# Harrypotterrrr/DVD-GAN

Hardware: AMD Instinct MI355X
Metric: clips/sec per G+Ds+Dt step, 48x64x64 UCF-101 synth (higher is better)
Workload: dtype bf16; 1 GPU; UCF-101-shaped 101-class 48x64x64 clips, G+Ds+Dt hinge step, ch=32, k_sample=8, batch 64/GPU (BASELINE configs[1]); global_batch=64, parallelism=dp1

## Files before the change

dvd_gan_amd/csrc/conv_wgrad.hip:

```cpp
#include "conv_common.h"
#include "prof.h"
#include <cstdlib>
#include <type_traits>

namespace {

struct WgK {
    const char* x; const char* dy; float* dw;
    int M, C, ldx, Cin_real, Cout, Cy, ldy;
    int T, H, W, logH, logW, Hin, Win;
    int kt, kh, kw, up2, relu_in;
    int tiles_co, tiles_ci, rows_per_split;
    long long s_co, s_ci, s_tap;
    size_t x_bytes, dy_bytes;
    int maxshift, xcd_remap;
    float* dbias;
    float* wsb;
    float* ws;
    int fold, cout_f;
};

template <typename G>
__host__ __device__ __forceinline__ size_t ws_tile_off(size_t slice, G gx, int bx, int kw, int t, int tile_elems) { return ((slice * gx + bx) * kw + t) * (size_t)tile_elems; }
template <typename G>
__host__ __device__ __forceinline__ size_t ws_slice_stride(G gx, int kw, int tile_elems) { return ws_tile_off(1, gx, 0, kw, 0, tile_elems); }
template <typename N>
__host__ __device__ __forceinline__ size_t ws_bias_off(size_t slice, N n, int i, int BMc) { return (slice * n + i) * BMc; }

__device__ __forceinline__ void xcd_block_remap(const WgK& p, int& bx, int& bz) {
    bx = blockIdx.x; bz = blockIdx.z;
    if (p.xcd_remap) {
        const int gx = gridDim.x, total = gx * gridDim.z, lin = bx + gx * bz;
        const int xcd = lin & 7, qd = total >> 3, rr = total & 7;
        const int lp = (xcd < rr ? xcd * (qd + 1) : rr * (qd + 1) + (xcd - rr) * qd) + (lin >> 3);
        bz = lp / gx; bx = lp - bz * gx;
    }
}
__device__ __forceinline__ void bf16x8_unpack(const u32x4& r, float (&v)[8]) {
    v[0] = __uint_as_float(r.x << 16); v[1] = __uint_as_float(r.x & 0xffff0000u);
    v[2] = __uint_as_float(r.y << 16); v[3] = __uint_as_float(r.y & 0xffff0000u);
    v[4] = __uint_as_float(r.z << 16); v[5] = __uint_as_float(r.z & 0xffff0000u);
    v[6] = __uint_as_float(r.w << 16); v[7] = __uint_as_float(r.w & 0xffff0000u);
}
#define WG_BIAS_FINISH(CPRA, RPPA, NV, TAB, TO_WS, N, I)                                                                \
    do {                                                                                                                \
        __syncthreads();                                                                                                \
        if (tid < CPRA) {                                                                                               \
            for (int k = 0; k < NV; ++k) {                                                                              \
                float a = 0.f;                                                                                          \
                for (int r = 0; r < RPPA; ++r) a += TAB;                                                                \
                const int co = co0 + tid * NV + k;                                                                      \
                if (TO_WS) p.wsb[ws_bias_off(bz, N, I, BMc) + tid * NV + k] = a;                                        \
                else if (co < p.Cout && a != 0.f) atomicAdd(p.dbias + co, a);      \
            }                                                                                                           \
        }                                                                                                               \
        __syncthreads();                                                                                                \
    } while (0)
#define WG_TILE_TAIL(ACC, ROW0, COL0, KW_, T, TAP)                                                                      \
    do {                                                                                                                \
        _Pragma("unroll") for (int r = 0; r < 16; ++r)                                                                  \
            ep[((r & 3) + 8 * (r >> 2) + 4 * (lane >> 5)) * 32 + (lane & 31)] = ACC[r];                                 \
        __builtin_amdgcn_s_waitcnt(0xc07f);                                                                             \
        __builtin_amdgcn_wave_barrier();                                                                                \
        const int ci = ci0 + COL0 + (lane & 31);                                                                        \
        const int cob = co0 + ROW0 + (lane >> 5);                                                                       \
        const int wtap = TAP;                   \
        if (p.ws) {                                                                                                     \
            float* wt = p.ws + ws_tile_off(bz, gridDim.x, bx, KW_, T, BMc * BNc) + (size_t)(ROW0) * BNc + COL0;         \
            _Pragma("unroll 1") for (int j = 0; j < 16; ++j)                                                            \
                wt[(size_t)(2 * j + (lane >> 5)) * BNc + (lane & 31)] = ep[(2 * j + (lane >> 5)) * 32 + (lane & 31)];   \
        } else if (ci < p.Cin_real) {                                                                                   \
            float* dst = p.dw + ci * p.s_ci + wtap * p.s_tap;                                                           \
            _Pragma("unroll 1") for (int j = 0; j < 16; ++j) {                                                          \
                const int co = cob + 2 * j;                                                                             \
                const float v = ep[(2 * j + (lane >> 5)) * 32 + (lane & 31)];                                           \
                if (co < p.Cout && v != 0.f) atomicAdd(dst + co * p.s_co, v);                                           \
            }                                                                                                           \
        }                                                                                                               \
        __builtin_amdgcn_wave_barrier();                                                                                \
    } while (0)
template <typename T, int TA, int TB>
__global__ __launch_bounds__(NT) void conv_wgrad_kernel(WgK p) {
    constexpr bool kBf16 = sizeof(T) == 2;
    static_assert(kBf16 || (TA == 2 && TB == 2), "exact mode uses the 128 x 128 tile");
    constexpr int BKW = kBf16 ? 32 : 16;
    constexpr int BMc = TA * 64, BNc = TB * 64;
    constexpr int RSA = BMc * 2 + 64, RSB = BNc * 2 + 64;
    constexpr int TA_BYTES = kBf16 ? 32 * RSA : TILEB, TB_BYTES = kBf16 ? 32 * RSB : TILEB;
    __shared__ __attribute__((aligned(16))) char smem[2][TA_BYTES + TB_BYTES];
    const int tid = threadIdx.x, lane = tid & 63, wave = tid >> 6;
    const int wm = wave >> 1, wn = wave & 1;
    int bx, bz;
    xcd_block_remap(p, bx, bz);
    const int tiles = p.tiles_co * p.tiles_ci;
    const int tap = bx / tiles;
    const int rem = bx - tap * tiles;
    const int tco = rem / p.tiles_ci, tci = rem - tco * p.tiles_ci;
    const int co0 = tco * BMc, ci0 = tci * BNc;
    const int it = tap / (p.kh * p.kw), r2 = tap - it * p.kh * p.kw;
    const int iy = r2 / p.kw, ix = r2 - iy * p.kw;
    const int dt = it - (p.kt >> 1), dy_ = iy - (p.kh >> 1), dx = ix - (p.kw >> 1);
    const int m_begin = bz * p.rows_per_split;
    const int m_end = min(p.M, m_begin + p.rows_per_split);

    f32x16 acc[TA][TB];
    {
        const f32x16 zacc = {0.f, 0.f, 0.f, 0.f, 0.f, 0.f, 0.f, 0.f, 0.f, 0.f, 0.f, 0.f, 0.f, 0.f, 0.f, 0.f};
#pragma unroll
        for (int a = 0; a < TA; ++a)
#pragma unroll
            for (int b = 0; b < TB; ++b) acc[a][b] = zacc;
    }

    constexpr unsigned ESZ = sizeof(T);
    const int xbase_row = p.up2 ? (m_begin / (p.H * p.W)) * p.Hin * p.Win : max(0, m_begin - p.maxshift);
    const size_t xbase_b = (size_t)xbase_row * p.ldx * ESZ, ybase_b = (size_t)m_begin * p.ldy * ESZ;
    const size_t xleft = p.x_bytes - xbase_b, yleft = p.dy_bytes > ybase_b ? p.dy_bytes - ybase_b : 0;
    const __amdgpu_buffer_rsrc_t rx = __builtin_amdgcn_make_buffer_rsrc(
        (void*)(p.x + xbase_b), 0, xleft > 0xfffffffeull ? 0xfffffffeu : (unsigned)xleft, 0x00020000);
    const __amdgpu_buffer_rsrc_t rdy = __builtin_amdgcn_make_buffer_rsrc(
        (void*)(p.dy + ybase_b), 0, yleft > 0xfffffffeull ? 0xfffffffeu : (unsigned)yleft, 0x00020000);
    const int delta = (dt * p.H + dy_) * p.W + dx;
    auto xoff = [&](int m, unsigned chan_bytes, bool cvalid) __attribute__((always_inline)) -> unsigned {
        int fm, ym, xm;
        grid_pos(m, p.H, p.W, p.logH, p.logW, fm, ym, xm);
        const int xx = xm + dx, yy = ym + dy_;
        int tt = dt;
        if (p.kt > 1) tt += fm % p.T;
        const bool ok = cvalid && m < m_end && (unsigned)yy < (unsigned)p.H && (unsigned)xx < (unsigned)p.W &&
                        (unsigned)tt < (unsigned)p.T;
        int row = m + delta;
        if (p.up2) row = ((fm + dt) * p.Hin + (yy >> 1)) * p.Win + (xx >> 1);
        return ok ? (unsigned)(row - xbase_row) * ((unsigned)p.ldx * ESZ) + chan_bytes : 0xffffffffu;
    };
    auto yoff = [&](int m, unsigned chan_bytes, bool cvalid) __attribute__((always_inline)) -> unsigned {
        return (cvalid && m < m_end) ? (unsigned)(m - m_begin) * ((unsigned)p.ldy * ESZ) + chan_bytes : 0xffffffffu;
    };

    if constexpr (kBf16) {
        constexpr int CPRA = BMc / 8, RPPA = NT / CPRA, NPA = 32 / RPPA;
        constexpr int CPRB = BNc / 8, RPPB = NT / CPRB, NPB = 32 / RPPB;
        const int rra = tid / CPRA, cka = tid % CPRA, rrb = tid / CPRB, ckb = tid % CPRB;
        const int cy = co0 + cka * 8, cx = ci0 + ckb * 8;
        const bool cyv = cy < p.Cy, cxv = cx < p.C;
// ... 386 lines not shown
                xoffs[kb][hl][t] = TA_BYTES + wn * XHALF + fr * 64 + fcol2;
            }
    const int aoff = frow * RSA + fcol2 + (wm * 64) * 2;
    auto mma1 = [&](const char* st) __attribute__((always_inline)) {
        constexpr int NU = 2 * KW;
        bf16x8 fa[2][2], fb[NU];
        auto ldA = [&](int kb) __attribute__((always_inline)) {
#pragma unroll
            for (int a = 0; a < 2; ++a) {
                const char* pz = st + aoff + kb * 16 * RSA + a * 64;
                fa[kb][a] = tr2(pz, pz + 4 * RSA);
            }
        };
        auto ldB = [&](int u) __attribute__((always_inline)) {
            const int kb = u / KW, t = u % KW;
            if constexpr (UP2) fb[u] = tr2(st + xoffs[kb][0][t], st + xoffs[kb][1][t]);
            else fb[u] = tr2(st + xoffs[kb][0][0] + t * 64, st + xoffs[kb][1][0] + t * 64);
        };
        ldA(0); ldB(0); ldB(1);
        __builtin_amdgcn_sched_barrier(0);
#pragma unroll
        for (int u = 0; u < NU; ++u) {
            if (u + 2 < NU) ldB(u + 2);
            if (u == KW - 2) ldA(1);
            const int kb = u / KW, t = u % KW;
            acc[0][t] = __builtin_amdgcn_mfma_f32_32x32x16_bf16(fa[kb][0], fb[u], acc[0][t], 0, 0, 0);
            acc[1][t] = __builtin_amdgcn_mfma_f32_32x32x16_bf16(fa[kb][1], fb[u], acc[1][t], 0, 0, 0);
            __builtin_amdgcn_sched_barrier(0);
        }
    };
    auto mma = [&](int buf) __attribute__((always_inline)) {
#pragma unroll
        for (int s_ = 0; s_ < NS; ++s_) mma1(&smem[buf * STAGE + s_ * SUB]);
    };
    if (m_begin < m_end) {
        const bool late = NWAVE == 8 && NS == 2 && wave >= 4;
        gload(m_begin);
        lstore(0);
        if (late) gload(m_begin + 32 * NS);
        __builtin_amdgcn_s_waitcnt(0xc07f);
        __builtin_amdgcn_s_barrier();
        int buf = 0;
        for (int mk = m_begin; mk < m_end; mk += 32 * NS, buf ^= 1) {
            if (!late) {
                gload(mk + 32 * NS);
                mma(buf);
                lstore(buf ^ 1);
            } else {
                mma1(&smem[buf * STAGE]);
                lstore(buf ^ 1);
                gload(mk + 2 * 32 * NS);
                mma1(&smem[buf * STAGE + (NS - 1) * SUB]);
            }
            __builtin_amdgcn_s_waitcnt(0xc07f);
            __builtin_amdgcn_s_barrier();
        }
        __builtin_amdgcn_s_waitcnt(0x0070);
    }
    if (do_bias) {
        float* red = reinterpret_cast<float*>(&smem[0]);
#pragma unroll
        for (int k = 0; k < 8; ++k) red[tid * 8 + k] = bs[k];
        WG_BIAS_FINISH(CPRA, RPPA, 8, red[(r * CPRA + tid) * 8 + k], spread, gridDim.x, bx);
    }
    float* ep = reinterpret_cast<float*>(&smem[0]) + wave * (32 * 32);
#pragma unroll
    for (int a = 0; a < 2; ++a)
#pragma unroll
        for (int t = 0; t < KW; ++t)
            WG_TILE_TAIL(acc[a][t], wm * 64 + a * 32, wn * 32, KW, t, irow * KW + t);
}
template <int I, int N, typename F>
__device__ __forceinline__ void static_for(F&& f) {
    if constexpr (I < N) {
        f(std::integral_constant<int, I>{});
        static_for<I + 1, N>(f);
    }
}
template <bool V>
__device__ __forceinline__ void mfma_pinned(f32x16& c, const bf16x8& a, const bf16x8& b) {
    if constexpr (V) asm volatile("v_mfma_f32_32x32x16_bf16 %0, %1, %2, %0" : "+v"(c) : "v"(a), "v"(b));
    else asm volatile("v_mfma_f32_32x32x16_bf16 %0, %1, %2, %0" : "+a"(c) : "v"(a), "v"(b));
}

#ifndef DVD_EXP_ROW4
#define DVD_EXP_ROW4 0
#endif
template <int KW, int AW, int BW, int WCO, int WCI, bool RELU, int DEPTH = 2, bool FOLD = false>
__global__ __launch_bounds__(256) void conv_wgrad_row4_kernel(WgK p) {
    constexpr bool BLDS = KW == 3 && AW * BW * KW > 16 && DEPTH >= 2;
    static_assert(WCO * WCI == 4, "four waves, one per SIMD");
    constexpr int NTt = 256, BMc = WCO * AW * 32, NHB = WCI * BW, BNc = NHB * 32;
    constexpr int RSA = BMc * 2 + 64;
    constexpr int TA_BYTES = 32 * RSA;
    constexpr int XROWS = KW == 5 ? 64 : 48, XHALF = XROWS * 64, TB_BYTES = NHB * XHALF;
    constexpr int SUB = TA_BYTES + TB_BYTES;
    constexpr int EPIB = 4 * 32 * 32 * 4, REDB = NTt * 8 * 4;
    constexpr int LDSB0 = 3 * SUB > EPIB ? (3 * SUB > REDB ? 3 * SUB : REDB) : (EPIB > REDB ? EPIB : REDB);
    constexpr int LDSB = LDSB0 + (BLDS ? REDB : 0);
    __shared__ __attribute__((aligned(16))) char smem[LDSB];
    const int tid = threadIdx.x, lane = tid & 63, wave = tid >> 6;
    const int wm = wave / WCI, wn = wave % WCI;
    int bx = blockIdx.x, bz = blockIdx.z;
    if (p.xcd_remap) {
        const int gx = gridDim.x, total = gx * gridDim.z, lin = bx + gx * bz;
        const int xcd = lin & 7, qd = total >> 3, rr = total & 7;
        const int lp = (xcd < rr ? xcd * (qd + 1) : rr * (qd + 1) + (xcd - rr) * qd) + (lin >> 3);
        bz = lp / gx; bx = lp - bz * gx;
    }
    const int tiles = p.tiles_co * p.tiles_ci;
    const int irow = bx / tiles;
    const int rem = bx - irow * tiles;
    const int tco = rem / p.tiles_ci, tci = rem - tco * p.tiles_ci;
    const int co0 = tco * BMc, ci0 = tci * BNc;
    constexpr int pad = KW >> 1;
    static_assert(!FOLD || (KW == 3 && BMc == 128), "the folded form runs on the 3-tap 128-channel tile");
    const int it = FOLD ? 0 : irow / KW, iy = FOLD ? irow : irow - it * KW;
    const int dyl = FOLD ? ((co0 / p.cout_f) >> 1) - 1 + irow : iy - pad, dtl = FOLD ? 0 : it - (p.kt >> 1);
    const int m_begin = bz * p.rows_per_split;
    const int m_end = min(p.M, m_begin + p.rows_per_split);

    f32x16 acc[AW][BW][KW];
    {
        const f32x16 zacc = {0.f, 0.f, 0.f, 0.f, 0.f, 0.f, 0.f, 0.f, 0.f, 0.f, 0.f, 0.f, 0.f, 0.f, 0.f, 0.f};
#pragma unroll
        for (int a = 0; a < AW; ++a)
#pragma unroll
            for (int b = 0; b < BW; ++b)
#pragma unroll
                for (int t = 0; t < KW; ++t) acc[a][b][t] = zacc;
    }
    const int xbase_row = max(0, m_begin - p.maxshift);
    const int ybase_row = FOLD ? 4 * m_begin - 2 * (p.W > 32 ? m_begin & (p.W - 1) : 0) : m_begin;
    const size_t xbase_b = (size_t)xbase_row * p.ldx * 2, ybase_b = (size_t)ybase_row * p.ldy * 2;
    const size_t xleft = p.x_bytes - xbase_b, yleft = p.dy_bytes > ybase_b ? p.dy_bytes - ybase_b : 0;
    const __amdgpu_buffer_rsrc_t rx = __builtin_amdgcn_make_buffer_rsrc(
        (void*)(p.x + xbase_b), 0, xleft > 0xfffffffeull ? 0xfffffffeu : (unsigned)xleft, 0x00020000);
    const __amdgpu_buffer_rsrc_t rdy = __builtin_amdgcn_make_buffer_rsrc(
        (void*)(p.dy + ybase_b), 0, yleft > 0xfffffffeull ? 0xfffffffeu : (unsigned)yleft, 0x00020000);
    const int segw = min(p.W, 32), logsegw = min(p.logW, 5);
    const int fpr = segw + KW - 1, frows = (32 >> logsegw) * fpr;
    constexpr int CPRA = BMc / 8, RPPA = NTt / CPRA, NPA = 32 / RPPA;
    const int rra = tid / CPRA, cka = tid % CPRA;
    const int cy = co0 + cka * 8;
    const bool cyv = cy < p.Cy;
    constexpr int CPX = NHB * 4;
    constexpr int NXL = (XROWS * CPX + NTt - 1) / NTt;
    constexpr int NOPS = NPA + NXL;
    constexpr bool XFULL = NXL * NTt == XROWS * CPX;
    int xa[NXL];
    static_assert(NTt % CPX == 0, "chunk i of a thread sits NTt / CPX footprint rows below chunk i - 1");
    const int xdst0 = ((tid % CPX) >> 2) * XHALF + (tid / CPX) * 64 + ((tid % CPX) & 3) * 16;
    unsigned xld[NXL];
    bool xv[NXL];
    const bool twofr = (32 >> logsegw) > p.H;
    const bool wide = p.W > 32;
    const unsigned ldx2 = (unsigned)p.ldx * 2, ldy2 = (unsigned)p.ldy * 2;
#pragma unroll
    for (int i = 0; i < NXL; ++i) {
        const int q = tid + i * NTt, row = q / CPX, c8 = q % CPX;
        const int seg = row / fpr, j = row - seg * fpr;
        const int cx = ci0 + c8 * 8;
        const int fo = twofr ? seg >> p.logH : 0, yl = twofr ? seg & (p.H - 1) : seg;
        const int xya = yl + dyl, xxa = j - pad;
        xa[i] = wide ? xxa : xya;
        xv[i] = row < frows && cx < p.C && (wide || (unsigned)xxa < (unsigned)p.W);
        const int delta = (fo << (p.logW + p.logH)) + (xya << p.logW) + xxa;
        xld[i] = (unsigned)delta * ldx2 + (unsigned)cx * 2;
    }
    unsigned yld = (unsigned)rra * ldy2 + (unsigned)cy * 2;
    unsigned ystep = (unsigned)RPPA * ldy2;
    if constexpr (FOLD) {
        static_assert(!FOLD || RPPA == 16, "16 rows per staging pass");
        const int ph = cy / p.cout_f, c = cy - ph * p.cout_f, W2 = 2 * p.W;
        yld = (unsigned)(((rra >> logsegw) * 2 + (ph >> 1)) * W2 + 2 * (rra & (segw - 1)) + (ph & 1)) * ldy2 + (unsigned)c * 2;
        ystep = (unsigned)(segw == 32 ? 32 : (16 >> logsegw) * 2 * W2) * ldy2;
    }
    const int dt_rows = p.kt > 1 ? dtl << (p.logW + p.logH) : 0;
    u32x4 R[DEPTH][NOPS];
    struct Geo { int sval; unsigned xoff, yoff; bool tok, ytok; };
    const unsigned slim = wide ? p.W : p.H;
    auto geo_part = [&](Geo& g, int mk, int part) __attribute__((always_inline)) {
        if (part == 0) {
            const int x0 = mk & (p.W - 1), y = twofr ? 0 : (mk >> p.logW) & (p.H - 1);
            g.sval = wide ? x0 : y;
            g.ytok = mk < m_end;
            g.tok = g.ytok && (!wide || (unsigned)(y + dyl) < (unsigned)p.H);
        } else if (part == 1) {
            if (p.kt > 1) {
                const int tt = (mk >> (p.logW + p.logH)) % p.T + dtl;
                g.tok = g.tok && (unsigned)tt < (unsigned)p.T;
            }
        } else if (part == 2) {
            g.xoff = (unsigned)(mk + dt_rows - xbase_row) * ldx2;
        } else {
            if constexpr (FOLD) g.yoff = (unsigned)(4 * mk - 2 * (wide ? mk & (p.W - 1) : 0) - ybase_row) * ldy2;
            else g.yoff = (unsigned)(mk - m_begin) * ldy2;
        }
    };
    auto geo = [&](int mk) __attribute__((always_inline)) -> Geo {
        Geo g;
#pragma unroll
        for (int part = 0; part < 4; ++part) geo_part(g, mk, part);
        return g;
    };
    auto load_op = [&](int op, const Geo& g, u32x4 (&R)[NOPS]) __attribute__((always_inline)) {
        if (op < NPA) {
            const unsigned off = (cyv && g.ytok) ? yld + g.yoff + (unsigned)op * ystep : 0xffffffffu;
            R[op] = __builtin_amdgcn_raw_buffer_load_b128(rdy, off, 0, 0);
        } else {
            const int i = op - NPA;
            const bool ok = xv[i] && g.tok && (unsigned)(g.sval + xa[i]) < slim;
            const unsigned off = ok ? xld[i] + g.xoff : 0xffffffffu;
            R[op] = __builtin_amdgcn_raw_buffer_load_b128(rx, off, 0, 0);
        }
    };
    const bool spread = p.ws != nullptr;
    const bool do_bias = p.dbias != nullptr && dtl == 0 && (spread || (dyl == 0 && tci == 0));
    const int nshare = spread ? (FOLD ? 2 : KW) * p.tiles_ci : 1, myshare = spread ? iy * p.tiles_ci + tci : 0;
    int bphase = 0;
    float bs[8] = {0.f, 0.f, 0.f, 0.f, 0.f, 0.f, 0.f, 0.f};
    float* btab = reinterpret_cast<float*>(&smem[BLDS ? LDSB0 : 0]) + tid;
    if (BLDS && do_bias) {
#pragma unroll
        for (int k = 0; k < 8; ++k) btab[k * NTt] = 0.f;
    }
    constexpr bool ST64 = KW == 5;
    typedef __attribute__((ext_vector_type(2))) unsigned u32x2;
    auto store_op = [&](int op, char* st, bool mine, const u32x4 (&R)[NOPS], int half = -1) __attribute__((always_inline)) {
        if (half >= 0) {
            const u32x4 v = (RELU && op >= NPA) ? relu16_bf16(R[op]) : R[op];
            const u32x2 h2 = half ? u32x2{v.z, v.w} : u32x2{v.x, v.y};
            char* dst = op < NPA ? st + (rra + op * RPPA) * RSA + cka * 16 : st + TA_BYTES + xdst0 + (op - NPA) * (NTt / CPX) * 64;
            if (op < NPA || XFULL || tid + (op - NPA) * NTt < XROWS * CPX) *reinterpret_cast<u32x2*>(dst + half * 8) = h2;
            if (half == 1 || op >= NPA || !mine) return;
            float v8[8];
            bf16x8_unpack(R[op], v8);
#pragma unroll
            for (int k = 0; k < 8; ++k) {
                if constexpr (BLDS) __hip_atomic_fetch_add(btab + k * NTt, v8[k], __ATOMIC_RELAXED, __HIP_MEMORY_SCOPE_WORKGROUP);
                else bs[k] += v8[k];
            }
            return;
        }
        if (op < NPA) {
            *reinterpret_cast<u32x4*>(st + (rra + op * RPPA) * RSA + cka * 16) = R[op];
            if (mine) {
                float v[8];
                bf16x8_unpack(R[op], v);
#pragma unroll
                for (int k = 0; k < 8; ++k) {
                    if constexpr (BLDS) __hip_atomic_fetch_add(btab + k * NTt, v[k], __ATOMIC_RELAXED, __HIP_MEMORY_SCOPE_WORKGROUP);
                    else bs[k] += v[k];
                }
            }
        } else {
            const int i = op - NPA;
            if (XFULL || tid + i * NTt < XROWS * CPX)
                *reinterpret_cast<u32x4*>(st + TA_BYTES + xdst0 + i * (NTt / CPX) * 64) = RELU ? relu16_bf16(R[op]) : R[op];
        }
    };
    typedef __attribute__((ext_vector_type(4))) short s16x4;
    typedef __attribute__((ext_vector_type(8))) short s16x8;
    const int g16 = lane >> 4, i16 = lane & 15;
    const int frow = (g16 >> 1) * 8 + (i16 >> 2), fcol2 = ((g16 & 1) * 16 + (i16 & 3) * 4) * 2;
    auto tr2 = [&](const char* lo_, const char* hi_) __attribute__((always_inline)) -> bf16x8 {
        s16x4 lo = __builtin_amdgcn_ds_read_tr16_b64_v4i16((__attribute__((address_space(3))) s16x4*)lo_);
        s16x4 hi = __builtin_amdgcn_ds_read_tr16_b64_v4i16((__attribute__((address_space(3))) s16x4*)hi_);
        s16x8 f = __builtin_shufflevector(lo, hi, 0, 1, 2, 3, 4, 5, 6, 7);
        return __builtin_bit_cast(bf16x8, f);
    };
    const int fr0 = (frow >> logsegw) * fpr + (frow & (segw - 1));
    const int hlstep = (segw >= 8 ? 4 : fpr) * 64;
    const int kbstep = ((16 >> logsegw) * fpr + (16 & (segw - 1))) * 64;
    const int xoff0 = TA_BYTES + wn * BW * XHALF + fr0 * 64 + fcol2;
    const int aoff = frow * RSA + fcol2 + (wm * AW * 32) * 2;
    constexpr int UPK = KW * BW, NU = 2 * UPK;
    constexpr bool PIN = AW * BW * KW > 16;
    constexpr int UB = NU - 2;
    constexpr int RING = NU % 3 == 0 ? 3 : 5;
    static_assert(NU % RING == 0, "B fragment ring");
    bf16x8 fa[AW], fb[RING];
    auto ldA = [&](const char* st, int kb, int a) __attribute__((always_inline)) {
        const char* pz = st + aoff + kb * 16 * RSA + a * 64;
        fa[a] = tr2(pz, pz + 4 * RSA);
    };
    auto ldB = [&](const char* st, int u, int slot) __attribute__((always_inline)) {
        const int kb = u / UPK, t = (u % UPK) / BW, b = u % BW;
        const char* pz = st + xoff0 + kb * kbstep + t * 64 + b * XHALF;
        fb[slot] = tr2(pz, pz + hlstep);
    };
    if (m_begin < m_end) {
        {
            const Geo g0 = geo(m_begin);
#pragma unroll
            for (int op = 0; op < NOPS; ++op) load_op(op, g0, R[0]);
            const bool mine = do_bias && bphase == myshare;
            if (++bphase == nshare) bphase = 0;
#pragma unroll
            for (int op = 0; op < NOPS; ++op) store_op(op, &smem[0], mine, R[0]);
#pragma unroll
            for (int d = 0; d < DEPTH; ++d) {
                const Geo g1 = geo(m_begin + 32 * (d + 1));
#pragma unroll
                for (int op = 0; op < NOPS; ++op) load_op(op, g1, R[d]);
            }
            __builtin_amdgcn_s_waitcnt(0xc07f);
            __builtin_amdgcn_s_barrier();
#pragma unroll
            for (int a = 0; a < AW - 1; ++a) ldA(&smem[0], 0, a);
            ldB(&smem[0], 0, 0);
            ldB(&smem[0], 1, 1);
        }
        char* rd = &smem[0];
        char* nx = &smem[SUB];
        char* fr_ = &smem[2 * SUB];
        static_assert(AW == 4, "slot plan written for four A fragments per wave");
        Geo gl = geo(m_begin + 32 * (DEPTH + 1));
        for (int mk0 = m_begin; mk0 < m_end; mk0 += 32 * DEPTH) {
          static_for<0, DEPTH>([&](auto D_) __attribute__((always_inline)) {
            constexpr int dset = decltype(D_)::value;
            const int mk = mk0 + 32 * dset;
            const bool mine = do_bias && bphase == myshare;
            if (++bphase == nshare) bphase = 0;
            Geo gn = gl;
            __builtin_amdgcn_sched_barrier(0);
            static_for<0, NU * AW>([&](auto S_) __attribute__((always_inline)) {
                constexpr int s = decltype(S_)::value, u = s / AW, a = s % AW;
                constexpr int kb = u / UPK, t = (u % UPK) / BW, b = u % BW;
                if constexpr (u == UB && a == 0) {
                    __builtin_amdgcn_s_waitcnt(0xc07f);
                    if (!(DVD_EXP_ROW4 & 4)) __builtin_amdgcn_s_barrier();
                }
                if constexpr (a == 0) {
                    if (u + 2 < NU) ldB(rd, u + 2, (u + 2) % RING);
                    else ldB(nx, u + 2 - NU, (u + 2) % RING);
                }
                if constexpr (a == 1 || (ST64 && a == 2)) {
#pragma unroll
                    for (int op = 0; op < NOPS; ++op)
                        if ((op * UB) / NOPS == u && !(DVD_EXP_ROW4 & 2)) {
                            if constexpr (ST64) store_op(op, nx, mine, R[dset], a - 1);
                            else store_op(op, nx, mine, R[dset]);
                        }
                }
                if constexpr (u == UPK - 1 && a >= 1) ldA(rd, 1, a - 1);
                if constexpr (u == UPK && a == 0) ldA(rd, 1, AW - 1);
                if constexpr (u == NU - 1 && a >= 1) ldA(nx, 0, a - 1);
                if constexpr (u == 0 && a == 0) ldA(rd, 0, AW - 1);
                if constexpr (a == AW - 1) {
#pragma unroll
                    for (int op = 0; op < NOPS; ++op)
                        if ((op * UB) / NOPS == u && !(DVD_EXP_ROW4 & 1)) load_op(op, gl, R[dset]);
                }
                if constexpr (u == UB - 1 && a == AW - 1) geo_part(gn, mk + 32 * (DEPTH + 2), 0);
                if constexpr (u == UB && a >= 1) geo_part(gn, mk + 32 * (DEPTH + 2), a);
                if constexpr (PIN) mfma_pinned<((a * BW + b) * KW + t >= 16)>(acc[a][b][t], fa[a], fb[u % RING]);
                else acc[a][b][t] = __builtin_amdgcn_mfma_f32_32x32x16_bf16(fa[a], fb[u % RING], acc[a][b][t], 0, 0, 0);
                __builtin_amdgcn_sched_barrier(0);
            });
            gl = gn;
            char* t_ = rd; rd = nx; nx = fr_; fr_ = t_;
          });
        }
        __builtin_amdgcn_s_waitcnt(0x0070);
        if constexpr (PIN) asm volatile("s_nop 15\n\ts_nop 15" ::: "memory");
        __syncthreads();
    }
    if (do_bias) {
        if constexpr (!BLDS) {
#pragma unroll
            for (int k = 0; k < 8; ++k) btab[k * NTt] = bs[k];
        }
        WG_BIAS_FINISH(CPRA, RPPA, 8, btab[k * NTt + r * CPRA], spread, gridDim.x, bx);
    }
    float* ep = reinterpret_cast<float*>(&smem[0]) + wave * (32 * 32);
#pragma unroll
    for (int a = 0; a < AW; ++a)
#pragma unroll
        for (int b = 0; b < BW; ++b)
#pragma unroll
            for (int t = 0; t < KW; ++t)
                WG_TILE_TAIL(acc[a][b][t], (wm * AW + a) * 32, (wn * BW + b) * 32, KW, t, irow * KW + t);
}
#undef WG_BIAS_FINISH
#undef WG_TILE_TAIL
__device__ __forceinline__ f32x4 slice_sum4(const float* ws, int nslice, size_t stride, size_t off) {
    f32x4 a = {0.f, 0.f, 0.f, 0.f};
    int z = 0;
    for (; z + 4 <= nslice; z += 4) {
        f32x4 v[4];
#pragma unroll
        for (int j = 0; j < 4; ++j) v[j] = *reinterpret_cast<const f32x4*>(ws + (size_t)(z + j) * stride + off);
#pragma unroll
        for (int j = 0; j < 4; ++j) a += v[j];
    }
    for (; z < nslice; ++z) a += *reinterpret_cast<const f32x4*>(ws + (size_t)z * stride + off);
    return a;
}
__device__ __forceinline__ void wg_store4(float* d, long long s_ci, int ci, int Cin_real, const f32x4& a, int overwrite) {
#pragma unroll
    for (int j = 0; j < 4; ++j)
        if (ci + j < Cin_real) d[j * s_ci] = overwrite ? a[j] : d[j * s_ci] + a[j];
}
template <typename F>
__device__ __forceinline__ float block_sum_32x32(int nitem, F&& item) {
    __shared__ float red[32][33];
    const int c = threadIdx.x & 31, l = threadIdx.x >> 5;
    float a = 0.f;
    for (int i = l; i < nitem; i += 32 * 8) {
        float v[8];
#pragma unroll
        for (int u = 0; u < 8; ++u) v[u] = i + 32 * u < nitem ? item(i + 32 * u) : 0.f;
#pragma unroll
        for (int u = 0; u < 8; ++u) a += v[u];
    }
    red[l][c] = a;
    __syncthreads();
    if (l == 0)
        for (int j = 1; j < 32; ++j) a += red[j][c];
    return a;
}

struct WgRowRedK { const float* ws; float* dw; int nslice, gx, tiles_co, tiles_ci, BMc, BNc, KW, Cout, Cin_real; long long s_co, s_ci, s_tap; int overwrite; };
__global__ void wgrad_row_reduce_kernel(WgRowRedK p) {
    const int tile = p.BMc * p.BNc, tile_elems = p.KW * tile;
    const long long i = ((long long)blockIdx.x * blockDim.x + threadIdx.x) * 4;
    if (i >= (long long)p.gx * tile_elems) return;
    const int bx = (int)(i / tile_elems), e = (int)(i - (long long)bx * tile_elems);
    const int t = e / tile, e2 = e - t * tile;
    const int r = e2 / p.BNc, c = e2 - r * p.BNc;
    const int tiles = p.tiles_co * p.tiles_ci;
    const int iy = bx / tiles, rem = bx - iy * tiles;
    const int tco = rem / p.tiles_ci, tci = rem - tco * p.tiles_ci;
    const int co = tco * p.BMc + r, ci = tci * p.BNc + c;
    if (co >= p.Cout || ci >= p.Cin_real) return;
    const f32x4 a = slice_sum4(p.ws, p.nslice, ws_slice_stride(p.gx, p.KW, tile), ws_tile_off(0, p.gx, bx, p.KW, t, tile) + e2);
    wg_store4(p.dw + co * p.s_co + ci * p.s_ci + (iy * p.KW + t) * p.s_tap, p.s_ci, ci, p.Cin_real, a, p.overwrite);
}

struct WgBiasRedK { const float* wsb; float* dbias; int nslice, gx, tiles_co, tiles_ci, KW, kt, BMc, Cout; };
__global__ __launch_bounds__(1024) void wgrad_row_bias_reduce_kernel(WgBiasRedK p) {
    const int gpt = p.BMc / 32;
    const int tco = blockIdx.x / gpt, cg = blockIdx.x - tco * gpt;
    const int c = threadIdx.x & 31;
    const int tiles = p.tiles_co * p.tiles_ci, per = p.KW * p.tiles_ci;
    const int irow0 = (p.kt >> 1) * p.KW;
    const float a = block_sum_32x32(p.nslice * per, [&](int i) __attribute__((always_inline)) -> float {
        const int bz = i / per, r = i - bz * per;
        const int iy = r / p.tiles_ci, tci = r - iy * p.tiles_ci;
        const int bx = (irow0 + iy) * tiles + tco * p.tiles_ci + tci;
        return p.wsb[ws_bias_off(bz, p.gx, bx, p.BMc) + cg * 32 + c];
    });
    const int co = tco * p.BMc + cg * 32 + c;
    if (threadIdx.x < 32 && co < p.Cout) p.dbias[co] += a;
}

__global__ __launch_bounds__(1024) void wgrad_bias_reduce_kernel(const float* wsb, float* dbias, int nslice, int tiles_co, int BMc, int Cout) {
    __shared__ float red[16][64];
    const int col = threadIdx.x & 63, q = threadIdx.x >> 6, co = blockIdx.x * 64 + col;
    float a = 0.f;
    if (co < Cout) {
        const int tco = co / BMc, c = co - tco * BMc;
#pragma unroll 4
        for (int z = q; z < nslice; z += 16) a += wsb[ws_bias_off(z, tiles_co, tco, BMc) + c];
    }
    red[q][col] = a;
    __syncthreads();
    if (q == 0 && co < Cout) {
// ... 143 lines not shown
    return cap;
}
static void wg_choose_split(const dvd_wgrad_desc* d, WgPlan& pl) {
    const bool automatic = d->msplit < 1;
    const long long M = pl.p.M, base = pl.base();
    long long msplit = d->msplit;
    if (automatic) {
        const long long cap = wg_split_cap(pl);
        msplit = wg_split_target(pl);
        if (msplit > cap) msplit = cap;
        const int per_cu = (pl.family != WG_TAP && (pl.bm == 256 || pl.bn == 128)) ? 1 : (pl.family == WG_ROW && pl.bm == 64) ? 3 : 2;
        const long long conc = WG_CUS * per_cu;
        if (base * msplit > conc) {
            const long long rounds = (base * msplit + conc / 2) / conc;
            const long long ms2 = rounds * conc / base;
            if (ms2 >= 1 && ms2 <= cap) msplit = ms2;
        }
    }
    long long rows = (M + msplit - 1) / msplit;
    const long long ldy_eff = pl.fold ? 4ll * d->ldy : d->ldy;
    const long long rowcap = (1ll << 31) / ((d->ldx > ldy_eff ? d->ldx : ldy_eff) * pl.esz);
    if (rows > rowcap) rows = rowcap;
    rows = (rows + 31) / 32 * 32;
    if (rows < 32) rows = 32;
    msplit = (M + rows - 1) / rows;
    const long long wg = base * msplit;
    if (automatic && pl.family == WG_ROW4 && wg > WG_CUS && wg % WG_CUS > 0 && wg % WG_CUS < 192) {
        const long long ms2 = ((wg + WG_CUS - 1) / WG_CUS * WG_CUS) / base;
        if (ms2 > msplit && M / ms2 >= 2048) {
            rows = ((M + ms2 - 1) / ms2 + 31) / 32 * 32;
            msplit = (M + rows - 1) / rows;
        }
    }
    pl.msplit = msplit;
    pl.p.rows_per_split = (int)rows;
    pl.grid = dim3((unsigned)base, 1, (unsigned)msplit);
}

static WgPlan wgrad_plan(const dvd_wgrad_desc* d, bool may_fold) {
    WgPlan pl{};
    auto plan1 = [&pl](const dvd_wgrad_desc* q, bool fold) {
        int rc = wg_fill_request(q, pl);
        if (rc == DVD_OK) rc = wg_choose_tile(q, fold, pl);
        if (rc == DVD_OK) wg_choose_split(q, pl);
        return rc;
    };
    pl.rc = DVD_E_SHAPE;
    if (may_fold && d && d->up2 && d->dtype == DVD_BF16 && d->kt == 1 && d->kh == 3 && d->kw == 3 && d->T == 1 &&
        d->Cout % 64 == 0 && d->Cy >= d->Cout && !((d->H | d->W) & 1)) {
        dvd_wgrad_desc e = *d;
        e.H = d->H / 2; e.W = d->W / 2; e.up2 = 0;
        e.Cout = e.Cy = 4 * d->Cout;
        pl.rc = plan1(&e, true);
        if (pl.rc == DVD_OK) {
            const size_t M4 = (size_t)d->frames * d->T * d->H * d->W;
            pl.p.dy_bytes = ((M4 - 1) * (size_t)d->ldy + d->Cy) * 2;
            pl.p.fold = 1; pl.p.cout_f = d->Cout;
        }
    }
    if (pl.rc != DVD_OK) pl.rc = plan1(d, false);
    if (pl.rc != DVD_OK) return pl;
    pl.kw_tile = pl.family == WG_TAP ? 1 : d->kw;
    pl.tile_floats = (long long)ws_tile_off(pl.msplit, pl.grid.x, 0, pl.kw_tile, 0, pl.bm * pl.bn);
    pl.bias_floats = (long long)ws_bias_off(pl.msplit, pl.family == WG_TAP ? (unsigned)pl.p.tiles_co : pl.grid.x, 0, pl.bm);
    return pl;
}

extern "C" long long dvd_conv_wgrad_ws_floats(const dvd_wgrad_desc* d) {
    if (const long long thin = dvd_wgrad_thin_ws_floats(d)) return thin;
    const WgPlan pl = wgrad_plan(d, true);
    if (pl.rc != DVD_OK || (pl.msplit <= 1 && !pl.fold)) return 0;
    return pl.total();
}

namespace {

template <int WM, int KW, bool UP2 = false, int NH = 2>
void launch_row(const WgPlan& pl, hipStream_t st) {
    if (pl.p.relu_in) conv_wgrad_row_kernel<WM, KW, true, UP2, NH><<<pl.grid, WM * NH * 64, 0, st>>>(pl.p);
    else conv_wgrad_row_kernel<WM, KW, false, UP2, NH><<<pl.grid, WM * NH * 64, 0, st>>>(pl.p);
}
template <int KW, int AW, int BW, int WCO, int WCI, int DEPTH, bool FOLD = false>
void launch_row4(const WgPlan& pl, hipStream_t st) {
    if (pl.p.relu_in) conv_wgrad_row4_kernel<KW, AW, BW, WCO, WCI, true, DEPTH, FOLD><<<pl.grid, 256, 0, st>>>(pl.p);
    else conv_wgrad_row4_kernel<KW, AW, BW, WCO, WCI, false, DEPTH, FOLD><<<pl.grid, 256, 0, st>>>(pl.p);
}

constexpr unsigned wg_key(WgFamily family, int bm, int bn, int kw, int up2, int depth, int fold, int f32 = 0) {
    return (unsigned)family | (bm / 64) << 2 | (bn / 64) << 5 | kw << 8 | up2 << 11 | depth << 12 | fold << 14 | f32 << 15;
}

bool wg_launch(const WgPlan& pl, hipStream_t st) {
    const bool tap = pl.family == WG_TAP;
    switch (wg_key(pl.family, pl.bm, pl.bn, tap ? 0 : pl.p.kw, tap ? 0 : pl.p.up2 != 0, pl.depth, pl.fold, tap && pl.esz == 4)) {
    case wg_key(WG_TAP,  256, 128, 0, 0, 0, 0):    conv_wgrad_kernel<bf16_t, 4, 2><<<pl.grid, NT, 0, st>>>(pl.p); break;
    case wg_key(WG_TAP,  128, 256, 0, 0, 0, 0):    conv_wgrad_kernel<bf16_t, 2, 4><<<pl.grid, NT, 0, st>>>(pl.p); break;
    case wg_key(WG_TAP,  128, 128, 0, 0, 0, 0):    conv_wgrad_kernel<bf16_t, 2, 2><<<pl.grid, NT, 0, st>>>(pl.p); break;
    case wg_key(WG_TAP,  128, 128, 0, 0, 0, 0, 1): conv_wgrad_kernel<float, 2, 2><<<pl.grid, NT, 0, st>>>(pl.p); break;
    case wg_key(WG_ROW,   64,  64, 3, 0, 0, 0):    launch_row<1, 3>(pl, st); break;
    case wg_key(WG_ROW,   64,  64, 5, 0, 0, 0):    launch_row<1, 5>(pl, st); break;
    case wg_key(WG_ROW,  128,  64, 3, 0, 0, 0):    launch_row<2, 3>(pl, st); break;
    case wg_key(WG_ROW,  128,  64, 5, 0, 0, 0):    launch_row<2, 5>(pl, st); break;
    case wg_key(WG_ROW,  256,  64, 3, 0, 0, 0):    launch_row<4, 3>(pl, st); break;
    case wg_key(WG_ROW,  256,  64, 5, 0, 0, 0):    launch_row<4, 5>(pl, st); break;
    case wg_key(WG_ROW,   64,  64, 3, 1, 0, 0):    launch_row<1, 3, true>(pl, st); break;
    case wg_key(WG_ROW,  128,  64, 3, 1, 0, 0):    launch_row<2, 3, true>(pl, st); break;
    case wg_key(WG_ROW,  256,  64, 3, 1, 0, 0):    launch_row<4, 3, true>(pl, st); break;
    case wg_key(WG_ROW,  128, 128, 3, 0, 0, 0):    launch_row<2, 3, false, 4>(pl, st); break;
    case wg_key(WG_ROW,  128, 128, 5, 0, 0, 0):    launch_row<2, 5, false, 4>(pl, st); break;
    case wg_key(WG_ROW4, 256, 128, 3, 0, 1, 0):    launch_row4<3, 4, 2, 2, 2, 1>(pl, st); break;
    case wg_key(WG_ROW4, 256, 128, 3, 0, 2, 0):    launch_row4<3, 4, 2, 2, 2, 2>(pl, st); break;
    case wg_key(WG_ROW4, 128, 128, 3, 0, 2, 0):    launch_row4<3, 4, 1, 1, 4, 2>(pl, st); break;
    case wg_key(WG_ROW4, 128, 128, 3, 0, 2, 1):    launch_row4<3, 4, 1, 1, 4, 2, true>(pl, st); break;
    case wg_key(WG_ROW4, 256,  64, 5, 0, 2, 0):    launch_row4<5, 4, 1, 2, 2, 2>(pl, st); break;
    case wg_key(WG_ROW4, 128, 128, 5, 0, 2, 0):    launch_row4<5, 4, 1, 1, 4, 2>(pl, st); break;
    default: return false;
    }
    return true;
}

}

extern "C" int dvd_conv_wgrad(const dvd_wgrad_desc* d, void* stream) {
    WgPlan pl = wgrad_plan(d, d && d->ws != nullptr);
    if (pl.rc != DVD_OK) return pl.rc;
    WgK& p = pl.p;
    hipStream_t st = (hipStream_t)stream;
    const int ntaps = d->kt * d->kh * d->kw, nslice = (int)pl.msplit, gx = (int)pl.grid.x;
    const long long Mreal = (long long)d->frames * d->T * d->H * d->W;
    if (d->ws && dvd_wgrad_thin_ws_floats(d)) {
        if (d->overwrite && (d->s_tap != 1 || d->s_ci != ntaps || d->s_co != (long long)d->Cin_real * ntaps)) return DVD_E_ARG;
        ProfScope prof(1, 2.0 * (double)Mreal * d->Cout * d->Cin_real * ntaps, stream, (int)Mreal, d->C, d->Cout, ntaps, 0, d->relu_in << 1);
        prof.r.variant = 3;
        return dvd_wgrad_thin(d, stream);
    }
    if (d->ws && (pl.msplit > 1 || pl.fold)) {
        p.ws = d->ws;
        p.wsb = d->ws + pl.tile_floats;
    }
    const int overwrite = d->overwrite != 0;
    if (overwrite) {
        if (d->s_tap != 1 || d->s_ci != ntaps || d->s_co != (long long)d->Cin_real * ntaps) return DVD_E_ARG;
        if (!p.ws && hipMemsetAsync(d->dw, 0, (size_t)d->Cout * d->Cin_real * ntaps * sizeof(float), st) != hipSuccess)
            return DVD_E_LAUNCH;
    }
    ProfScope prof(1, 2.0 * (double)Mreal * d->Cout * d->Cin_real * ntaps, stream, (int)Mreal, d->C, d->Cout, ntaps, nslice,
                   d->up2 | (d->relu_in << 1));
    prof.r.variant = pl.family == WG_ROW4 ? 4 : pl.family == WG_ROW ? 1 : 2;
    if (!wg_launch(pl, st)) return DVD_E_SHAPE;
    if (!p.ws) return launch_status();
    if (pl.fold) {
        WgFoldRedK r{p.ws, p.dw, nslice, gx, p.tiles_ci, d->Cout, p.Cin_real, p.s_co, p.s_ci, p.s_tap, overwrite};
        wgrad_fold_reduce_kernel<<<cdiv(9ll * d->Cout * ((p.Cin_real + 3) / 4), 256), 256, 0, st>>>(r);
        if (p.dbias) {
            WgFoldBiasK b{p.wsb, p.dbias, nslice, gx, p.tiles_ci, d->Cout};
            wgrad_fold_bias_reduce_kernel<<<cdiv(d->Cout, 32), 1024, 0, st>>>(b);
        }
        return launch_status();
    }
    WgRowRedK r{p.ws, p.dw, nslice, gx, p.tiles_co, p.tiles_ci, pl.bm, pl.bn, pl.kw_tile, p.Cout, p.Cin_real, p.s_co, p.s_ci, p.s_tap, overwrite};
    const long long n = pl.tile_floats / nslice;
    wgrad_row_reduce_kernel<<<cdiv(n / 4, 256), 256, 0, st>>>(r);
    if (p.dbias) {
        if (pl.family == WG_TAP) wgrad_bias_reduce_kernel<<<cdiv(p.Cout, 64), 1024, 0, st>>>(p.wsb, p.dbias, nslice, p.tiles_co, pl.bm, p.Cout);
        else {
            WgBiasRedK b{p.wsb, p.dbias, nslice, gx, p.tiles_co, p.tiles_ci, d->kw, d->kt, pl.bm, p.Cout};
            wgrad_row_bias_reduce_kernel<<<p.tiles_co * (pl.bm / 32), 1024, 0, st>>>(b);
        }
// ... 4 lines not shown
```

Baseline: 146.7 clips/s.

## Use 16x16x32 MFMA tiles in row4 wgrad kernel with new LDS layout

Adds an MF16 variant of the row4 weight-gradient kernel that splits each 32x32 accumulator into four 16x16 quadrants computed with v_mfma_f32_16x16x32_bf16. The LDS staging layout (X row block width, padding) and fragment addressing change to match, and global loads are split into a precomputed-offset step and a separate issue step interleaved into the MFMA schedule. The aim is to spread the MFMA stream and memory ops more finely and reduce LDS bank conflicts. The cost is more MFMA instructions, twice as many A fragment reads, and a new epilogue layout that has to be correct. It is enabled by default for most row4 configurations (DVD_WG_MF16=15), with the mask excluding some.

```diff
diff --git a/dvd_gan_amd/csrc/conv_wgrad.hip b/dvd_gan_amd/csrc/conv_wgrad.hip
--- a/dvd_gan_amd/csrc/conv_wgrad.hip
+++ b/dvd_gan_amd/csrc/conv_wgrad.hip
@@ -60,6 +60,16 @@
     do {                                                                                                                \
         _Pragma("unroll") for (int r = 0; r < 16; ++r)                                                                  \
             ep[((r & 3) + 8 * (r >> 2) + 4 * (lane >> 5)) * 32 + (lane & 31)] = ACC[r];                                 \
+        WG_TILE_OUT(ROW0, COL0, KW_, T, TAP);                                                                           \
+    } while (0)
+#define WG_TILE_TAIL16(Q, ROW0, COL0, KW_, T, TAP)                                                                      \
+    do {                                                                                                                \
+        _Pragma("unroll") for (int r = 0; r < 16; ++r)                                                                  \
+            ep[(16 * (r >> 3) + 4 * (lane >> 4) + (r & 3)) * 32 + 16 * ((r >> 2) & 1) + (lane & 15)] = Q[r >> 3][(r >> 2) & 1][r & 3]; \
+        WG_TILE_OUT(ROW0, COL0, KW_, T, TAP);                                                                           \
+    } while (0)
+#define WG_TILE_OUT(ROW0, COL0, KW_, T, TAP)                                                                            \
+    do {                                                                                                                \
         __builtin_amdgcn_s_waitcnt(0xc07f);                                                                             \
         __builtin_amdgcn_wave_barrier();                                                                                \
         const int ci = ci0 + COL0 + (lane & 31);                                                                        \
@@ -612,18 +622,27 @@
     if constexpr (V) asm volatile("v_mfma_f32_32x32x16_bf16 %0, %1, %2, %0" : "+v"(c) : "v"(a), "v"(b));
     else asm volatile("v_mfma_f32_32x32x16_bf16 %0, %1, %2, %0" : "+a"(c) : "v"(a), "v"(b));
 }
+template <bool V>
+__device__ __forceinline__ void mfma_pinned(f32x4& c, const bf16x8& a, const bf16x8& b) {
+    if constexpr (V) asm volatile("v_mfma_f32_16x16x32_bf16 %0, %1, %2, %0" : "+v"(c) : "v"(a), "v"(b));
+    else asm volatile("v_mfma_f32_16x16x32_bf16 %0, %1, %2, %0" : "+a"(c) : "v"(a), "v"(b));
+}
+struct WgAcc16 { f32x4 q[2][2]; };
+#ifndef DVD_WG_MF16
+#define DVD_WG_MF16 15
+#endif
 
 #ifndef DVD_EXP_ROW4
 #define DVD_EXP_ROW4 0
 #endif
-template <int KW, int AW, int BW, int WCO, int WCI, bool RELU, int DEPTH = 2, bool FOLD = false>
+template <int KW, int AW, int BW, int WCO, int WCI, bool RELU, int DEPTH = 2, bool FOLD = false, bool MF16 = false>
 __global__ __launch_bounds__(256) void conv_wgrad_row4_kernel(WgK p) {
     constexpr bool BLDS = KW == 3 && AW * BW * KW > 16 && DEPTH >= 2;
     static_assert(WCO * WCI == 4, "four waves, one per SIMD");
     constexpr int NTt = 256, BMc = WCO * AW * 32, NHB = WCI * BW, BNc = NHB * 32;
-    constexpr int RSA = BMc * 2 + 64;
+    constexpr int RSA = BMc * 2 + (MF16 ? 32 : 64);
     constexpr int TA_BYTES = 32 * RSA;
-    constexpr int XROWS = KW == 5 ? 64 : 48, XHALF = XROWS * 64, TB_BYTES = NHB * XHALF;
+    constexpr int XROWS = KW == 5 ? 64 : 48, XRB = MF16 ? 32 : 64, XBLK = XROWS * XRB + (MF16 ? 32 : 0), TB_BYTES = BNc * 2 / XRB * XBLK;
     constexpr int SUB = TA_BYTES + TB_BYTES;
     constexpr int EPIB = 4 * 32 * 32 * 4, REDB = NTt * 8 * 4;
     constexpr int LDSB0 = 3 * SUB > EPIB ? (3 * SUB > REDB ? 3 * SUB : REDB) : (EPIB > REDB ? EPIB : REDB);
@@ -650,15 +669,19 @@
     const int m_begin = bz * p.rows_per_split;
     const int m_end = min(p.M, m_begin + p.rows_per_split);
 
-    f32x16 acc[AW][BW][KW];
+    std::conditional_t<MF16, WgAcc16, f32x16> acc[AW][BW][KW];
     {
         const f32x16 zacc = {0.f, 0.f, 0.f, 0.f, 0.f, 0.f, 0.f, 0.f, 0.f, 0.f, 0.f, 0.f, 0.f, 0.f, 0.f, 0.f};
+        const f32x4 zq = {0.f, 0.f, 0.f, 0.f};
 #pragma unroll
         for (int a = 0; a < AW; ++a)
 #pragma unroll
             for (int b = 0; b < BW; ++b)
 #pragma unroll
-                for (int t = 0; t < KW; ++t) acc[a][b][t] = zacc;
+                for (int t = 0; t < KW; ++t) {
+                    if constexpr (MF16) acc[a][b][t] = WgAcc16{{{zq, zq}, {zq, zq}}};
+                    else acc[a][b][t] = zacc;
+                }
     }
     const int xbase_row = max(0, m_begin - p.maxshift);
     const int ybase_row = FOLD ? 4 * m_begin - 2 * (p.W > 32 ? m_begin & (p.W - 1) : 0) : m_begin;
@@ -680,7 +703,8 @@
     constexpr bool XFULL = NXL * NTt == XROWS * CPX;
     int xa[NXL];
     static_assert(NTt % CPX == 0, "chunk i of a thread sits NTt / CPX footprint rows below chunk i - 1");
-    const int xdst0 = ((tid % CPX) >> 2) * XHALF + (tid / CPX) * 64 + ((tid % CPX) & 3) * 16;
+    constexpr int XCB = XRB / 16;
+    const int xdst0 = ((tid % CPX) / XCB) * XBLK + (tid / CPX) * XRB + ((tid % CPX) % XCB) * 16;
     unsigned xld[NXL];
     bool xv[NXL];
     const bool twofr = (32 >> logsegw) > p.H;
@@ -708,14 +732,17 @@
     }
     const int dt_rows = p.kt > 1 ? dtl << (p.logW + p.logH) : 0;
     u32x4 R[DEPTH][NOPS];
-    struct Geo { int sval; unsigned xoff, yoff; bool tok, ytok; };
+    struct Geo { int sval, y; unsigned xoff, yoff; bool tok, ytok; };
     const unsigned slim = wide ? p.W : p.H;
     auto geo_part = [&](Geo& g, int mk, int part) __attribute__((always_inline)) {
         if (part == 0) {
             const int x0 = mk & (p.W - 1), y = twofr ? 0 : (mk >> p.logW) & (p.H - 1);
             g.sval = wide ? x0 : y;
+            g.y = y;
+        }
+        if (part == (MF16 ? 4 : 0)) {
             g.ytok = mk < m_end;
-            g.tok = g.ytok && (!wide || (unsigned)(y + dyl) < (unsigned)p.H);
+            g.tok = g.ytok && (!wide || (unsigned)(g.y + dyl) < (unsigned)p.H);
         } else if (part == 1) {
             if (p.kt > 1) {
                 const int tt = (mk >> (p.logW + p.logH)) % p.T + dtl;
@@ -731,7 +758,10 @@
     auto geo = [&](int mk) __attribute__((always_inline)) -> Geo {
         Geo g;
 #pragma unroll
-        for (int part = 0; part < 4; ++part) geo_part(g, mk, part);
+        for (int part = 0; part < 4; ++part) {
+            geo_part(g, mk, part);
+            if (MF16 && part == 0) geo_part(g, mk, 4);
+        }
         return g;
     };
     auto load_op = [&](int op, const Geo& g, u32x4 (&R)[NOPS]) __attribute__((always_inline)) {
@@ -745,6 +775,15 @@
             R[op] = __builtin_amdgcn_raw_buffer_load_b128(rx, off, 0, 0);
         }
     };
+    auto load_off = [&](int op, const Geo& g) __attribute__((always_inline)) -> unsigned {
+        if (op < NPA) return (cyv && g.ytok) ? yld + g.yoff + (unsigned)op * ystep : 0xffffffffu;
+        const int i = op - NPA;
+        const bool ok = xv[i] && g.tok && (unsigned)(g.sval + xa[i]) < slim;
+        return ok ? xld[i] + g.xoff : 0xffffffffu;
+    };
+    auto load_at = [&](int op, unsigned off, u32x4 (&R)[NOPS]) __attribute__((always_inline)) {
+        R[op] = __builtin_amdgcn_raw_buffer_load_b128(op < NPA ? rdy : rx, off, 0, 0);
+    };
     const bool spread = p.ws != nullptr;
     const bool do_bias = p.dbias != nullptr && dtl == 0 && (spread || (dyl == 0 && tci == 0));
     const int nshare = spread ? (FOLD ? 2 : KW) * p.tiles_ci : 1, myshare = spread ? iy * p.tiles_ci + tci : 0;
@@ -761,9 +800,11 @@
         if (half >= 0) {
             const u32x4 v = (RELU && op >= NPA) ? relu16_bf16(R[op]) : R[op];
             const u32x2 h2 = half ? u32x2{v.z, v.w} : u32x2{v.x, v.y};
-            char* dst = op < NPA ? st + (rra + op * RPPA) * RSA + cka * 16 : st + TA_BYTES + xdst0 + (op - NPA) * (NTt / CPX) * 64;
+            char* dst = op < NPA ? st + (rra + op * RPPA) * RSA + cka * 16 : st + TA_BYTES + xdst0 + (op - NPA) * (NTt / CPX) * XRB;
             if (op < NPA || XFULL || tid + (op - NPA) * NTt < XROWS * CPX) *reinterpret_cast<u32x2*>(dst + half * 8) = h2;
-            if (half == 1 || op >= NPA || !mine) return;
+            if (half == 1 || op >= NPA) return;
+            if constexpr (MF16) { if (__builtin_expect(!mine, true)) return; }
+            else if (!mine) return;
             float v8[8];
             bf16x8_unpack(R[op], v8);
 #pragma unroll
@@ -775,7 +816,7 @@
         }
         if (op < NPA) {
             *reinterpret_cast<u32x4*>(st + (rra + op * RPPA) * RSA + cka * 16) = R[op];
-            if (mine) {
+            if (MF16 ? __builtin_expect(mine, false) : mine) {
                 float v[8];
                 bf16x8_unpack(R[op], v);
 #pragma unroll
@@ -787,13 +828,14 @@
         } else {
             const int i = op - NPA;
             if (XFULL || tid + i * NTt < XROWS * CPX)
-                *reinterpret_cast<u32x4*>(st + TA_BYTES + xdst0 + i * (NTt / CPX) * 64) = RELU ? relu16_bf16(R[op]) : R[op];
+                *reinterpret_cast<u32x4*>(st + TA_BYTES + xdst0 + i * (NTt / CPX) * XRB) = RELU ? relu16_bf16(R[op]) : R[op];
         }
     };
     typedef __attribute__((ext_vector_type(4))) short s16x4;
     typedef __attribute__((ext_vector_type(8))) short s16x8;
     const int g16 = lane >> 4, i16 = lane & 15;
-    const int frow = (g16 >> 1) * 8 + (i16 >> 2), fcol2 = ((g16 & 1) * 16 + (i16 & 3) * 4) * 2;
+    const int frow = MF16 ? (g16 >> 1) * 16 + (g16 & 1) * 4 + (i16 >> 2) : (g16 >> 1) * 8 + (i16 >> 2);
+    const int fcol2 = MF16 ? (i16 & 3) * 8 : ((g16 & 1) * 16 + (i16 & 3) * 4) * 2;
     auto tr2 = [&](const char* lo_, const char* hi_) __attribute__((always_inline)) -> bf16x8 {
         s16x4 lo = __builtin_amdgcn_ds_read_tr16_b64_v4i16((__attribute__((address_space(3))) s16x4*)lo_);
         s16x4 hi = __builtin_amdgcn_ds_read_tr16_b64_v4i16((__attribute__((address_space(3))) s16x4*)hi_);
@@ -801,23 +843,24 @@
         return __builtin_bit_cast(bf16x8, f);
     };
     const int fr0 = (frow >> logsegw) * fpr + (frow & (segw - 1));
-    const int hlstep = (segw >= 8 ? 4 : fpr) * 64;
+    const int hlstep = MF16 ? ((8 >> logsegw) * fpr + (8 & (segw - 1))) * XRB : (segw >= 8 ? 4 : fpr) * 64;
     const int kbstep = ((16 >> logsegw) * fpr + (16 & (segw - 1))) * 64;
-    const int xoff0 = TA_BYTES + wn * BW * XHALF + fr0 * 64 + fcol2;
+    const int xoff0 = TA_BYTES + wn * BW * (64 / XRB) * XBLK + fr0 * XRB + fcol2;
     const int aoff = frow * RSA + fcol2 + (wm * AW * 32) * 2;
     constexpr int UPK = KW * BW, NU = 2 * UPK;
     constexpr bool PIN = AW * BW * KW > 16;
     constexpr int UB = NU - 2;
     constexpr int RING = NU % 3 == 0 ? 3 : 5;
     static_assert(NU % RING == 0, "B fragment ring");
-    bf16x8 fa[AW], fb[RING];
+    constexpr int NFA = MF16 ? 2 * AW : AW;
+    bf16x8 fa[NFA], fb[RING];
     auto ldA = [&](const char* st, int kb, int a) __attribute__((always_inline)) {
-        const char* pz = st + aoff + kb * 16 * RSA + a * 64;
-        fa[a] = tr2(pz, pz + 4 * RSA);
+        const char* pz = MF16 ? st + aoff + a * 32 : st + aoff + kb * 16 * RSA + a * 64;
+        fa[a] = tr2(pz, pz + (MF16 ? 8 : 4) * RSA);
     };
     auto ldB = [&](const char* st, int u, int slot) __attribute__((always_inline)) {
         const int kb = u / UPK, t = (u % UPK) / BW, b = u % BW;
-        const char* pz = st + xoff0 + kb * kbstep + t * 64 + b * XHALF;
+        const char* pz = MF16 ? st + xoff0 + (u / (2 * BW)) * XRB + (u % (2 * BW)) * XBLK : st + xoff0 + kb * kbstep + t * 64 + b * XBLK;
         fb[slot] = tr2(pz, pz + hlstep);
     };
     if (m_begin < m_end) {
@@ -838,7 +881,7 @@
             __builtin_amdgcn_s_waitcnt(0xc07f);
             __builtin_amdgcn_s_barrier();
 #pragma unroll
-            for (int a = 0; a < AW - 1; ++a) ldA(&smem[0], 0, a);
+            for (int a = 0; a < NFA - 1; ++a) ldA(&smem[0], 0, a);
             ldB(&smem[0], 0, 0);
             ldB(&smem[0], 1, 1);
         }
@@ -855,7 +898,46 @@
             if (++bphase == nshare) bphase = 0;
             Geo gn = gl;
             __builtin_amdgcn_sched_barrier(0);
-            static_for<0, NU * AW>([&](auto S_) __attribute__((always_inline)) {
+            unsigned lofs[2] = {0xffffffffu, 0xffffffffu};
+            if constexpr (MF16) static_for<0, NU * NFA>([&](auto S_) __attribute__((always_inline)) {
+                constexpr int s = decltype(S_)::value, u = s / NFA, a = s % NFA;
+                constexpr int t = u / (2 * BW), j = u % (2 * BW), b = j >> 1;
+                static_assert(NOPS <= (ST64 ? UB : 2 * UB), "at most one (two) staging chunks per unit");
+                if constexpr (u == UB && a == 0) {
+                    __builtin_amdgcn_s_waitcnt(0xc07f);
+                    if (!(DVD_EXP_ROW4 & 4)) __builtin_amdgcn_s_barrier();
+                }
+                if constexpr (a == 0) {
+                    if (u + 2 < NU) ldB(rd, u + 2, (u + 2) % RING);
+                    else ldB(nx, u + 2 - NU, (u + 2) % RING);
+                }
+                if constexpr (u < UB && (a == 2 || a == 4)) {
+#pragma unroll
+                    for (int op = 0; op < NOPS; ++op)
+                        if ((op * UB) / NOPS == u && !(DVD_EXP_ROW4 & 2)) {
+                            const bool second = op > 0 && ((op - 1) * UB) / NOPS == u;
+                            if constexpr (ST64) store_op(op, nx, mine, R[dset], (a - 2) >> 1);
+                            else if (second == (a == 4)) store_op(op, nx, mine, R[dset]);
+                        }
+                }
+                if constexpr (u == NU - 1 && a >= 1) ldA(nx, 0, a - 1);
+                if constexpr (u == 0 && a == 0) ldA(rd, 0, NFA - 1);
+                if constexpr (u < UB && (a == 3 || a == 5 || a == 6 || a == 7)) {
+#pragma unroll
+                    for (int op = 0; op < NOPS; ++op)
+                        if ((op * UB) / NOPS == u && !(DVD_EXP_ROW4 & 1)) {
+                            const int k2 = op > 0 && ((op - 1) * UB) / NOPS == u;
+                            if (a == (k2 ? 3 : 5)) lofs[k2] = load_off(op, gl);
+                            if (a == (k2 ? 7 : 6)) load_at(op, lofs[k2], R[dset]);
+                        }
+                }
+                if constexpr (u == UB - 2 && a == NFA - 1) geo_part(gn, mk + 32 * (DEPTH + 2), 0);
+                if constexpr (u == UB - 1 && a == NFA - 1) geo_part(gn, mk + 32 * (DEPTH + 2), 4);
+                if constexpr (u == UB && (a & 1) == 1 && a < 6) geo_part(gn, mk + 32 * (DEPTH + 2), (a >> 1) + 1);
+                mfma_pinned<((a / 2 * BW + b) * KW + t >= 16)>(acc[a / 2][b][t].q[a & 1][j & 1], fa[a], fb[u % RING]);
+                __builtin_amdgcn_sched_barrier(0);
+            });
+            else static_for<0, NU * AW>([&](auto S_) __attribute__((always_inline)) {
                 constexpr int s = decltype(S_)::value, u = s / AW, a = s % AW;
                 constexpr int kb = u / UPK, t = (u % UPK) / BW, b = u % BW;
                 if constexpr (u == UB && a == 0) {
@@ -894,7 +976,7 @@
           });
         }
         __builtin_amdgcn_s_waitcnt(0x0070);
-        if constexpr (PIN) asm volatile("s_nop 15\n\ts_nop 15" ::: "memory");
+        if constexpr (PIN || MF16) asm volatile("s_nop 15\n\ts_nop 15" ::: "memory");
         __syncthreads();
     }
     if (do_bias) {
@@ -910,11 +992,15 @@
 #pragma unroll
         for (int b = 0; b < BW; ++b)
 #pragma unroll
-            for (int t = 0; t < KW; ++t)
-                WG_TILE_TAIL(acc[a][b][t], (wm * AW + a) * 32, (wn * BW + b) * 32, KW, t, irow * KW + t);
+            for (int t = 0; t < KW; ++t) {
+                if constexpr (MF16) WG_TILE_TAIL16(acc[a][b][t].q, (wm * AW + a) * 32, (wn * BW + b) * 32, KW, t, irow * KW + t);
+                else WG_TILE_TAIL(acc[a][b][t], (wm * AW + a) * 32, (wn * BW + b) * 32, KW, t, irow * KW + t);
+            }
 }
 #undef WG_BIAS_FINISH
 #undef WG_TILE_TAIL
+#undef WG_TILE_TAIL16
+#undef WG_TILE_OUT
 __device__ __forceinline__ f32x4 slice_sum4(const float* ws, int nslice, size_t stride, size_t off) {
     f32x4 a = {0.f, 0.f, 0.f, 0.f};
     int z = 0;
@@ -1224,8 +1310,9 @@
 }
 template <int KW, int AW, int BW, int WCO, int WCI, int DEPTH, bool FOLD = false>
 void launch_row4(const WgPlan& pl, hipStream_t st) {
-    if (pl.p.relu_in) conv_wgrad_row4_kernel<KW, AW, BW, WCO, WCI, true, DEPTH, FOLD><<<pl.grid, 256, 0, st>>>(pl.p);
-    else conv_wgrad_row4_kernel<KW, AW, BW, WCO, WCI, false, DEPTH, FOLD><<<pl.grid, 256, 0, st>>>(pl.p);
+    constexpr bool MF16 = (DVD_WG_MF16 & (KW == 5 ? (BW == 1 && WCI == 2 ? 1 : 2) : FOLD ? 8 : AW * BW * KW > 16 ? 16 : 4)) != 0;
+    if (pl.p.relu_in) conv_wgrad_row4_kernel<KW, AW, BW, WCO, WCI, true, DEPTH, FOLD, MF16><<<pl.grid, 256, 0, st>>>(pl.p);
+    else conv_wgrad_row4_kernel<KW, AW, BW, WCO, WCI, false, DEPTH, FOLD, MF16><<<pl.grid, 256, 0, st>>>(pl.p);
 }
 
 constexpr unsigned wg_key(WgFamily family, int bm, int bn, int kw, int up2, int depth, int fold, int f32 = 0) {
```

Result: no change. 147.7 clips/s (median of 6 runs) (+0.7%).
